# LukasHedegaard/continual-skeletons

Measured on AMD Instinct MI355X. Metric: clips/sec (ST-GCN clip forward, NTU-60 shape; CoST-GCN online step reported under costgcn_online), higher is better.
Workload: dtype f32

## Files before the change

### continual-skeletons_amd/csrc/gcn.hip

```cpp
#include <type_traits>

#include "mfma_core.h"
#include "gcn_params.h"


template <int MT, int NJ>
__global__ __launch_bounds__(NTHREADS, 2) void gcn_stage_kernel(const GcnParams p) {
    constexpr int NT = 16384 / MT;
    constexpr int WM = MT / 64;
    constexpr int TPC = NTHREADS / NT;
    constexpr int KPT = KC / TPC;
    extern __shared__ __attribute__((aligned(16))) float smem[];
    const int V = p.V, R = p.R, EW = p.ell_w;
    float *Wl = smem;
    float *Xa = Wl + R * KC * MT;
    float *Bx = Xa + R * KC * NT;
    float *Lv = Bx + KC * p.ldb;
    int *Ls = reinterpret_cast<int *>(Lv + 3 * V * EW * (p.adj_per_frame ? p.lds_frames : 1));

    const int tid = threadIdx.x, lane = tid & 63, wave = __builtin_amdgcn_readfirstlane(tid >> 6);
    const int wm = wave % WM, wn = wave / WM;
    const int l31 = lane & 31, kh = lane >> 5;
    const unsigned wid = xcd_contiguous_id(blockIdx.x, gridDim.x);
    const int m0 = (int)(wid % p.mtiles) * MT, q0 = (int)((wid / p.mtiles) % p.qtiles) * NT;
// ... 155 lines not shown
        for (int g = 0; g < 16; ++g) {
            const float v0 = relu_nan(acc[mi][0][g] + bb[mi][g] + rv[0][mi][g]);
            const float v1 = relu_nan(acc[mi][1][g] + bb[mi][g] + rv[1][mi][g]);
            const auto sw = __builtin_amdgcn_permlane32_swap(__float_as_uint(v0), __float_as_uint(v1), false, false);
            acc[mi][0][g] = __uint_as_float(sw[0]);
            acc[mi][1][g] = __uint_as_float(sw[1]);
        }
    const int qb = q0 + wn * 64 + lane;
    const bool qv = qb < Q;
    if (full) {
        if (qv) {
            const unsigned qo = 4u * (unsigned)qb;
#pragma unroll
            for (int mi = 0; mi < 2; ++mi)
#pragma unroll
                for (int g = 0; g < 16; ++g) {
                    float *orow = oseg + (int64_t)(rbase + mi * 32 + (g & 3) + 8 * (g >> 2)) * p.y_chan_stride;
                    st_lane(orow, qo, acc[mi][0][g]);
                    st_lane(orow + 4 * p.y_chan_stride, qo, acc[mi][1][g]);
                }
        }
    } else {
#pragma unroll
        for (int mi = 0; mi < 2; ++mi)
#pragma unroll
            for (int g = 0; g < 16; ++g) {
                const int row0 = rbase + mi * 32 + (g & 3) + 8 * (g >> 2);
                if (qv && row0 < p.Cout) oseg[(int64_t)row0 * p.y_chan_stride + qb] = acc[mi][0][g];
                if (qv && row0 + 4 < p.Cout) oseg[(int64_t)(row0 + 4) * p.y_chan_stride + qb] = acc[mi][1][g];
            }
    }
}

template <int MT, bool CONVRES, int KCG_, bool PLAIN = false, bool SPLIT = false>
__global__ __launch_bounds__(NTHREADS, 3) void gcn_stage_sparse2_kernel(const GcnParams p) {
    constexpr int NT = 16384 / MT;
    constexpr int WM = MT / 64;
    constexpr int R = PLAIN ? 1 : (CONVRES ? 4 : 3);
    constexpr int M4 = MT / 4;
    constexpr int WB = (R * KCG_ * M4 + NTHREADS - 1) / NTHREADS;
    constexpr int RPW = KCG_ / (NTHREADS / 64);
    constexpr int NJ = MT == 128 ? 3 : 5;
    constexpr int NS = KCG_ / 2;
    constexpr int NH = NS / 2;
    static_assert(KCG_ % 8 == 0, "a chunk is a whole number of rows per wave");
    extern __shared__ __attribute__((aligned(16))) float smem[];
    const int V = p.V;
    const int wsz = R * KCG_ * MT, bsz = KCG_ * p.ldb, bufsz = wsz + bsz;

    const int tid = threadIdx.x, lane = tid & 63, wave = __builtin_amdgcn_readfirstlane(tid >> 6);
    const int wm = wave % WM, wn = wave / WM;
    const int l31 = lane & 31, kh = lane >> 5;
    const unsigned wid = xcd_contiguous_id(blockIdx.x, gridDim.x);
    const int m0 = (int)(wid % p.mtiles) * MT, q0 = (int)((wid / p.mtiles) % p.qtiles) * NT;
    const int segks = (int)(wid / (p.mtiles * p.qtiles));
    const int seg = SPLIT ? segks / p.ksplit : segks, ks = SPLIT ? segks % p.ksplit : 0;
    const int cb = SPLIT ? ks * p.cper : 0;
    const int Q = p.frames * V;
    const int qend = min(q0 + NT, Q);
    const int ta = div_magic(q0, p.vmagic), tb = div_magic(qend - 1, p.vmagic);
    const int span = (tb - ta + 1) * V;
    int eoff[2][6];
    float eval[2][6];
    int ioff[2];
#pragma unroll
    for (int ni = 0; ni < 2; ++ni) {
        const int q = min(q0 + wn * 64 + ni * 32 + l31, Q - 1);
        const int t = div_magic(q, p.vmagic);
        const int w = q - t * V, fb = (t - ta) * V;
        ioff[ni] = fb + w;
#pragma unroll
        for (int e = 0; e < 6; ++e) {
            const int r = e < 2 ? e : 2, k = e < 2 ? 0 : e - 2;
            const bool have = !PLAIN && k < p.ell_cnt[r];
            const int idx = PLAIN ? 0 : (r * V + w) * p.ell_w + min(k, p.ell_w - 1);
            eoff[ni][e] = fb + (have ? p.ell_src[idx] : 0);
            eval[ni][e] = have ? p.ell_val[idx] : 0.f;
        }
    }

    f32x16 acc[2][2];
#pragma unroll
    for (int a = 0; a < 2; ++a)
#pragma unroll
        for (int b = 0; b < 2; ++b)
#pragma unroll
            for (int g = 0; g < 16; ++g) acc[a][b][g] = 0.f;

    const float *seg_base = p.x + (int64_t)seg * p.x_seg_stride;
    const float *wbase = p.w + m0 + (size_t)cb * p.Mpad;
    f32x4 wv[WB];
    unsigned wgo[WB], wlo[WB];
#pragma unroll
    for (int u = 0; u < WB; ++u) {
        const int e = min(u * NTHREADS + tid, R * KCG_ * M4 - 1);
        const int row = e / M4, m4 = e % M4;
        wgo[u] = (unsigned)(((row / KCG_) * p.CinPad + (row % KCG_)) * p.Mpad + m4 * 4);
        wlo[u] = (unsigned)(e * 4);
    }
    constexpr int NJ4 = (NJ + 3) / 4;
    float bv[RPW][NJ];
    f32x4 bv4[RPW][NJ4];
    unsigned bgo[NJ], blo[NJ];
#pragma unroll
    for (int u = 0; u < NJ; ++u) {
        const int j = min(u * 64 + lane, span - 1);
        bgo[u] = (unsigned)(ta * V + j);
        blo[u] = (unsigned)j;
    }
    const int nvec = (span + 3) / 4;
    const bool vec = ta * V + 4 * nvec <= Q && p.Cin >= KCG_;
    unsigned bgo4[NJ4], blo4[NJ4];
#pragma unroll
    for (int u = 0; u < NJ4; ++u) {
        const int i = min(u * 64 + lane, nvec - 1);
        bgo4[u] = (unsigned)(ta * V + 4 * i);
        blo4[u] = (unsigned)(4 * i);
    }
    auto issue_one = [&](auto vtag, int i, int c0) {
        constexpr bool VEC = decltype(vtag)::value;
        constexpr int NX = VEC ? NJ4 : NJ;
        if (i < WB) {
            wv[i] = *reinterpret_cast<const f32x4 *>(wbase + (size_t)c0 * p.Mpad + wgo[i]);
        } else {
            const int rr = (i - WB) / NX, u = (i - WB) % NX;
            const int c = min(cb + c0 + wave + rr * (NTHREADS / 64), p.Cin - 1);
            const float *row = seg_base + (int64_t)c * p.x_chan_stride;
            if (VEC) bv4[rr][u] = *reinterpret_cast<const f32x4u *>(row + bgo4[u]);
            else bv[rr][u] = row[bgo[u]];
        }
    };
    auto commit = [&](auto vtag, float *buf) {
        constexpr bool VEC = decltype(vtag)::value;
        float *Wl = buf, *Bx = buf + wsz;
#pragma unroll
        for (int u = 0; u < WB; ++u) *reinterpret_cast<f32x4 *>(Wl + wlo[u]) = wv[u];
#pragma unroll
        for (int rr = 0; rr < RPW; ++rr) {
            float *dst = Bx + (wave + rr * (NTHREADS / 64)) * p.ldb;
            if (VEC) {
#pragma unroll
                for (int u = 0; u < NJ4; ++u) *reinterpret_cast<f32x4 *>(dst + blo4[u]) = bv4[rr][u];
            } else {
#pragma unroll
                for (int u = 0; u < NJ; ++u) dst[blo[u]] = bv[rr][u];
            }
        }
    };
    const int offA = wm * 64 + l31;
    auto mfma_step = [&](const float *buf, int s) {
        const float *Wl = buf, *Bx = buf + wsz;
        const int kk = 2 * s + kh;
        const float *bx = Bx + kk * p.ldb;
        float b[R][2];
#pragma unroll
        for (int ni = 0; ni < 2; ++ni) {
            if constexpr (PLAIN) {
                b[0][ni] = bx[ioff[ni]];
            } else {
                const float x0 = bx[eoff[ni][0]];
// ... 5 lines not shown
                s2 = fmaf(eval[ni][5], bx[eoff[ni][5]], s2);
                b[2][ni] = s2;
                if (CONVRES) b[R - 1][ni] = bx[ioff[ni]];
            }
        }
#pragma unroll
        for (int r = 0; r < R; ++r) {
            const float *wr = Wl + (r * KCG_ + kk) * MT + offA;
            const float a0 = wr[0], a1 = wr[32];
            acc[0][0] = __builtin_amdgcn_mfma_f32_32x32x2f32(a0, b[r][0], acc[0][0], 0, 0, 0);
            acc[0][1] = __builtin_amdgcn_mfma_f32_32x32x2f32(a0, b[r][1], acc[0][1], 0, 0, 0);
            acc[1][0] = __builtin_amdgcn_mfma_f32_32x32x2f32(a1, b[r][0], acc[1][0], 0, 0, 0);
            acc[1][1] = __builtin_amdgcn_mfma_f32_32x32x2f32(a1, b[r][1], acc[1][1], 0, 0, 0);
        }
    };

    const int nchunks = (SPLIT ? min(p.CinPad - cb, p.cper) : p.CinPad) / KCG_;
    auto k_loop = [&](auto vtag) {
        constexpr int NLX = WB + RPW * (decltype(vtag)::value ? NJ4 : NJ);
#pragma unroll
        for (int i = 0; i < NLX; ++i) issue_one(vtag, i, 0);
        commit(vtag, smem);
        if (nchunks > 1) {
#pragma unroll
            for (int i = 0; i < NLX; ++i) issue_one(vtag, i, KCG_);
        }
        __syncthreads();
        for (int c = 0; c + 1 < nchunks; ++c) {
            float *cur = smem + (c & 1) * bufsz, *oth = smem + ((c & 1) ^ 1) * bufsz;
            commit(vtag, oth);
            const int cnext = min(c + 2, nchunks - 1) * KCG_;
            __builtin_amdgcn_s_setprio(1);
#pragma unroll
            for (int s = 0; s < NS; ++s) {
                if (s < NH) {
#pragma unroll
                    for (int i = s * NLX / NH; i < (s + 1) * NLX / NH; ++i) issue_one(vtag, i, cnext);
                    __builtin_amdgcn_sched_barrier(0);
                }
                mfma_step(cur, s);
            }
            __builtin_amdgcn_s_setprio(0);
            __syncthreads();
        }
    };
    if (vec) k_loop(std::true_type{});
    else k_loop(std::false_type{});
    const float *last = smem + ((nchunks - 1) & 1) * bufsz;
    const int rbase = m0 + wm * 64;
    const bool full = p.fast_epi && m0 + MT <= p.Cout;
    const unsigned kh4 = 4u * (unsigned)kh;
    float *oseg = SPLIT ? p.part + (int64_t)(seg * p.ksplit + ks) * p.Cout * p.y_chan_stride : p.y + (int64_t)seg * p.y_seg_stride;
    const int qb = q0 + wn * 64 + lane;
    const bool qv = qb < Q;
    float bb[2][16], rv[2][2][16];
    auto load_half = [&](int mi) {
        if (SPLIT) {
#pragma unroll
            for (int g = 0; g < 16; ++g) bb[mi][g] = rv[0][mi][g] = rv[1][mi][g] = 0.f;
        } else if (full) {
#pragma unroll
            for (int g = 0; g < 16; ++g) bb[mi][g] = ld_lane(p.bias + (rbase + mi * 32 + (g & 3) + 8 * (g >> 2)), kh4 * 4u);
#pragma unroll
            for (int ni = 0; ni < 2; ++ni) {
                const unsigned lo = 4u * (kh4 * (unsigned)p.x_chan_stride + (unsigned)min(q0 + wn * 64 + ni * 32 + l31, Q - 1));
#pragma unroll
                for (int g = 0; g < 16; ++g) {
                    const float *rrow = seg_base + (int64_t)(rbase + mi * 32 + (g & 3) + 8 * (g >> 2)) * p.x_chan_stride;
                    rv[ni][mi][g] = (CONVRES || PLAIN) ? 0.f : ld_lane(rrow, lo);
                }
            }
        } else {
#pragma unroll
            for (int g = 0; g < 16; ++g) bb[mi][g] = p.bias[rbase + mi * 32 + 4 * kh + (g & 3) + 8 * (g >> 2)];
#pragma unroll
            for (int ni = 0; ni < 2; ++ni) {
                const int qc = min(q0 + wn * 64 + ni * 32 + l31, Q - 1);
#pragma unroll
                for (int g = 0; g < 16; ++g) {
                    const int co = rbase + mi * 32 + 4 * kh + (g & 3) + 8 * (g >> 2);
                    rv[ni][mi][g] = (CONVRES || PLAIN) ? 0.f : seg_base[(int64_t)min(co, p.Cout - 1) * p.x_chan_stride + qc];
                }
            }
        }
    };
    auto finish_half = [&](int mi) {
#pragma unroll
        for (int g = 0; g < 16; ++g) {
            float v0 = acc[mi][0][g] + bb[mi][g] + rv[0][mi][g];
            float v1 = acc[mi][1][g] + bb[mi][g] + rv[1][mi][g];
            if (!PLAIN && !SPLIT) { v0 = relu_nan(v0); v1 = relu_nan(v1); }
            const auto sw = __builtin_amdgcn_permlane32_swap(__float_as_uint(v0), __float_as_uint(v1), false, false);
            acc[mi][0][g] = __uint_as_float(sw[0]);
            acc[mi][1][g] = __uint_as_float(sw[1]);
        }
        if (full) {
            if (qv) {
                const unsigned qo = 4u * (unsigned)qb;
#pragma unroll
                for (int g = 0; g < 16; ++g) {
                    float *orow = oseg + (int64_t)(rbase + mi * 32 + (g & 3) + 8 * (g >> 2)) * p.y_chan_stride;
                    st_lane(orow, qo, acc[mi][0][g]);
                    st_lane(orow + 4 * p.y_chan_stride, qo, acc[mi][1][g]);
                }
            }
        } else {
#pragma unroll
            for (int g = 0; g < 16; ++g) {
                const int row0 = rbase + mi * 32 + (g & 3) + 8 * (g >> 2);
                if (qv && row0 < p.Cout) oseg[(int64_t)row0 * p.y_chan_stride + qb] = acc[mi][0][g];
                if (qv && row0 + 4 < p.Cout) oseg[(int64_t)(row0 + 4) * p.y_chan_stride + qb] = acc[mi][1][g];
            }
        }
    };
#pragma unroll
    for (int s = 0; s < NS; ++s) mfma_step(last, s);
    load_half(0);
    finish_half(0);
    load_half(1);
    finish_half(1);
}

template <int MT, bool CONVRES, int KC2, int OCC>
__global__ __launch_bounds__(NTHREADS, OCC) void gcn_stage_dense_kernel(const GcnParams p) {
    constexpr int NT = 16384 / MT;
    constexpr int WM = MT / 64;
    constexpr int R = CONVRES ? 4 : 3;
    constexpr int M4 = MT / 4;
    constexpr int WB = R * KC2 * M4 / NTHREADS;
    constexpr int WBU = (R * KC2 * M4 + NTHREADS - 1) / NTHREADS;
    extern __shared__ __attribute__((aligned(16))) float smem[];
    const int V = p.V, FT = p.lds_frames, ldbx = p.ldb;
    float *Wl = smem;
    float *Xa = Wl + R * KC2 * MT;
    float *Bx = Xa + 3 * KC2 * NT;
    float *Ladj = Bx + KC2 * ldbx;

    const int tid = threadIdx.x, lane = tid & 63, wave = __builtin_amdgcn_readfirstlane(tid >> 6);
    const int wm = wave % WM, wn = wave / WM;
    const int l31 = lane & 31, kh = lane >> 5;
    const unsigned wid = xcd_contiguous_id(blockIdx.x, gridDim.x);
    const int m0 = (int)(wid % p.mtiles) * MT, qt = (int)((wid / p.mtiles) % p.qtiles);
    const int seg = (int)(wid / (p.mtiles * p.qtiles));
    const int Q = p.frames * V;
    const int ta = qt * FT, q0 = ta * V;
    const int fcnt = min(FT, p.frames - ta);
    const int ncol = fcnt * V;
    (void)WB;

    {
        const float *gv = p.ell_val + (int64_t)seg * p.adj_seg_stride;
        for (int e = tid; e < 3 * V * V; e += NTHREADS) Ladj[e] = gv[e];
    }
    f32x16 acc[2][2];
#pragma unroll
    for (int a = 0; a < 2; ++a)
#pragma unroll
        for (int b = 0; b < 2; ++b)
#pragma unroll
            for (int g = 0; g < 16; ++g) acc[a][b][g] = 0.f;

    const float *seg_base = p.x + (int64_t)seg * p.x_seg_stride;
    const float *wbase = p.w + m0;
    f32x4 wv[WBU];
// ... 153 lines not shown
                }
            }
        } else {
#pragma unroll
            for (int g = 0; g < 16; ++g) {
                const int row0 = rbase + mi * 32 + (g & 3) + 8 * (g >> 2);
                if (qv && row0 < p.Cout) oseg[(int64_t)row0 * p.y_chan_stride + qb] = acc[mi][0][g];
                if (qv && row0 + 4 < p.Cout) oseg[(int64_t)(row0 + 4) * p.y_chan_stride + qb] = acc[mi][1][g];
            }
        }
    }
}

__global__ __launch_bounds__(256) void gcn_reduce_kernel(const GcnParams p) {
    const int Q = p.frames * p.V;
    const int64_t i = (int64_t)blockIdx.x * 256 + threadIdx.x;
    if (i >= (int64_t)p.Cout * Q) return;
    const int co = (int)(i / Q), q = (int)(i - (int64_t)co * Q), seg = blockIdx.y;
    float s = 0.f;
    for (int ks = 0; ks < p.ksplit; ++ks) s += p.part[((int64_t)(seg * p.ksplit + ks) * p.Cout + co) * p.y_chan_stride + q];
    s += p.bias[co];
    if (p.res_mode == CSK_RES_IDENTITY) s += p.x[(int64_t)seg * p.x_seg_stride + (int64_t)co * p.x_chan_stride + q];
    p.y[(int64_t)seg * p.y_seg_stride + (int64_t)co * p.y_chan_stride + q] = relu_nan(s);
}

static int gcn_stage_setup(const float *x, float *y, const float *w, const float *bias, const int32_t *ell_src, const float *ell_val,
                           const int32_t *ell_cnt, int ell_w, int64_t adj_seg_stride, int adj_per_frame, int n_seg, int c_in, int c_out,
                           int frames, int V, int64_t x_seg_stride, int64_t x_chan_stride, int64_t y_seg_stride, int64_t y_chan_stride,
                           int res_mode, int ksplit, float *partial, GcnParams *out, size_t *lds_out, bool *sparse_out) {
    if (n_seg <= 0 || c_in <= 0 || c_out <= 0 || frames <= 0 || V < 2 || V > 64) CSK_FAIL("gcn_stage: bad dims");
    if (ell_w < 1 || ell_w > V) CSK_FAIL("gcn_stage: ell_w must be in [1, V]");
    if (res_mode != CSK_RES_IDENTITY && res_mode != CSK_RES_CONV) CSK_FAIL("gcn_stage: res_mode must be identity or conv");
    if (res_mode == CSK_RES_IDENTITY && c_in != c_out) CSK_FAIL("gcn_stage: identity residual needs c_in == c_out");
    for (int i = 0; i < 3; ++i)
        if (ell_cnt[i] < 0 || ell_cnt[i] > ell_w) CSK_FAIL("gcn_stage: ell_cnt[%d] out of range", i);
    GcnParams &p = *out;
    p = gcn_params(x, y, w, bias, ell_src, ell_val, ell_cnt, ell_w, adj_seg_stride, c_in, c_out, frames, V, x_seg_stride,
                   x_chan_stride, y_seg_stride, y_chan_stride, res_mode, partial);
    p.dense = adj_seg_stride != 0 && ell_w == V && ell_cnt[0] == V && ell_cnt[1] == V && ell_cnt[2] == V;
    p.adj_per_frame = adj_per_frame != 0;
    if (p.adj_per_frame && !p.dense) CSK_FAIL("gcn_stage: per-frame adjacency must be dense (ell_w == V, ell_cnt == V)");
    const bool big = (p.Mpad % 128) == 0;
    const int MT = big ? 128 : 64, NT = 16384 / MT;
    const int max_dt = (NT + V - 2) / V;
    p.ldb = round_up((max_dt + 1) * V, 4);
    p.lds_frames = max_dt + 1;
    const size_t lds = (size_t)(p.R * KC * MT + p.R * KC * NT + KC * p.ldb + 3 * V * ell_w * (1 + (p.adj_per_frame ? p.lds_frames : 1))) * sizeof(float);
    if (lds > 160 * 1024) CSK_FAIL("gcn_stage: LDS tile %zu B exceeds 160 KiB", lds);
    const int Q = frames * V;
    if ((int64_t)frames * V >= (1 << 26)) CSK_FAIL("gcn_stage: frames*V too large for 32-bit position arithmetic");
    p.qtiles = (Q + NT - 1) / NT; p.mtiles = p.Mpad / MT;
    if ((int64_t)p.qtiles * p.mtiles * n_seg >= (1ll << 31)) CSK_FAIL("gcn_stage: grid too large");
    const bool sparse = adj_seg_stride == 0 && ell_cnt[0] <= 1 && ell_cnt[1] <= 1 && ell_cnt[2] <= 4 && p.ldb <= (big ? 192 : 320) &&
                        !csk_diag_flag("CSK_GCN_GENERAL");
    if (ksplit > 1 && !sparse) CSK_FAIL("gcn_stage_splitk: split-K is built for the skeleton-sparse kernel (shared adjacency, <= 1/1/4 non-zeros per column)");
    p.ksplit = split_ranges(p.CinPad, c_in, ksplit, 8, &p.cper);
    *lds_out = lds; *sparse_out = sparse;
    return 0;
}

static bool gcn16_candidate(const GcnParams &p, bool sparse) { return sparse && p.ksplit == 1; }

enum { ROUTE_UNIT = 1000000, ROUTE_SPARSE2 = 1, ROUTE_TILE16 = 2, ROUTE_DENSE2 = 3, ROUTE_DENSE128 = 4, ROUTE_GENERAL = 5 };
enum { ROUTE_SPLIT = 1 << 30, ROUTE_SPLIT_MT128 = 1 << 29, ROUTE_SPLIT_CONVRES = 1 << 28, ROUTE_SPLIT_RANGES_SHIFT = 23, ROUTE_SPLIT_CPER_MASK = (1 << 23) - 1 };
static int gcn_stage_route(const GcnParams &p, bool sparse, int n_seg) {
    const bool big = (p.Mpad % 128) == 0;
    const int MT = big ? 128 : 64, NT = 16384 / MT, V = p.V;
    if (p.ksplit > 1) {
        if (p.cper / 8 > ROUTE_SPLIT_CPER_MASK) CSK_FAIL("gcn_stage_splitk: %d channels per range exceed the split launch", p.cper);
        return ROUTE_SPLIT | (big ? ROUTE_SPLIT_MT128 : 0) | (p.R == 4 ? ROUTE_SPLIT_CONVRES : 0) | ((p.ksplit - 1) << ROUTE_SPLIT_RANGES_SHIFT) |
               (p.cper / 8);
    }
    if (gcn16_candidate(p, sparse)) {
        if (const int tile = csk_gcn16_tile(p, n_seg)) return ROUTE_TILE16 * ROUTE_UNIT + tile;
    }
    if (sparse) return ROUTE_SPARSE2 * ROUTE_UNIT + MT * 10 + (p.R == 4 ? 1 : 0);
    if (p.dense) {
        if (const int d2 = csk_gcn_dense2_route(p, n_seg)) return ROUTE_DENSE2 * ROUTE_UNIT + d2;
    }
    if (big && p.dense && !p.adj_per_frame && V >= 4 && V <= 32 && NT / V >= 1 && p.frames * (int64_t)V >= 4) {
        const int ft = NT / V;
        if ((int64_t)((p.frames + ft - 1) / ft) * p.mtiles * n_seg >= (1ll << 31)) CSK_FAIL("gcn_stage: grid too large");
        return ROUTE_DENSE128 * ROUTE_UNIT + (p.R == 4 ? 1 : 0);
    }
    const int nj = (p.ldb + 63) / 64;
    if (nj > (big ? 4 : 6)) CSK_FAIL("gcn_stage: activation tile of %d positions per channel exceeds the staged maximum", p.ldb);
    return ROUTE_GENERAL * ROUTE_UNIT + MT * 10 + (big ? (nj <= 3 ? 3 : 4) : (nj <= 5 ? 5 : 6));
}

static int gcn_stage_impl(const float *x, float *y, const float *w, const float *bias, const int32_t *ell_src,
                          const float *ell_val, const int32_t *ell_cnt, int ell_w, int64_t adj_seg_stride,
                          int adj_per_frame,
                          int n_seg, int c_in, int c_out, int frames, int V, int64_t x_seg_stride,
                          int64_t x_chan_stride, int64_t y_seg_stride, int64_t y_chan_stride, int res_mode,
                          int ksplit, float *partial, void *stream) {
    if (!x || !y || !w || !bias || !ell_src || !ell_val || !ell_cnt) CSK_FAIL("gcn_stage: null pointer");
    GcnParams p;
    size_t lds;
    bool sparse;
    if (const int rc = gcn_stage_setup(x, y, w, bias, ell_src, ell_val, ell_cnt, ell_w, adj_seg_stride, adj_per_frame, n_seg, c_in, c_out, frames,
                                       V, x_seg_stride, x_chan_stride, y_seg_stride, y_chan_stride, res_mode, ksplit, partial, &p, &lds, &sparse))
        return rc;
    const bool big = (p.Mpad % 128) == 0;
    const int MT = big ? 128 : 64, NT = 16384 / MT;
    const int Q = frames * V;
    dim3 grid(p.qtiles * p.mtiles * n_seg);
    const int route = gcn_stage_route(p, sparse, n_seg);
    if (route < 0) return route;
    const bool split = (route & ROUTE_SPLIT) != 0;
    const int family = split ? ROUTE_SPARSE2 : route / ROUTE_UNIT;
    if (family == ROUTE_TILE16) return csk_launch_gcn16(p, n_seg, stream);
    if (family == ROUTE_SPARSE2) {
        const int R = p.R;
        size_t lds2;
        void (*k)(GcnParams);
        lds2 = 2 * (size_t)(R * 8 * MT + 8 * p.ldb) * sizeof(float);
        if (split) {
            const bool big2 = (route & ROUTE_SPLIT_MT128) != 0, convres = (route & ROUTE_SPLIT_CONVRES) != 0;
            const int ranges = ((route >> ROUTE_SPLIT_RANGES_SHIFT) & 31) + 1;
            if ((int64_t)p.qtiles * p.mtiles * n_seg * ranges >= (1ll << 31)) CSK_FAIL("gcn_stage: grid too large");
            grid = dim3(p.qtiles * p.mtiles * n_seg * ranges);
            k = big2 ? (convres ? gcn_stage_sparse2_kernel<128, true, 8, false, true> : gcn_stage_sparse2_kernel<128, false, 8, false, true>)
                     : (convres ? gcn_stage_sparse2_kernel<64, true, 8, false, true> : gcn_stage_sparse2_kernel<64, false, 8, false, true>);
        } else {
            k = big ? (R == 4 ? gcn_stage_sparse2_kernel<128, true, 8> : gcn_stage_sparse2_kernel<128, false, 8>)
                    : (R == 4 ? gcn_stage_sparse2_kernel<64, true, 8> : gcn_stage_sparse2_kernel<64, false, 8>);
        }
        const int e = csk_ensure_lds((const void *)k, lds2);
        if (e) return e;
        hipLaunchKernelGGL(k, grid, dim3(NTHREADS), lds2, (hipStream_t)stream, p);
        if (split) {
            if (const int e2 = (int)hipGetLastError()) return e2;
            const int64_t work = (int64_t)c_out * Q;
            hipLaunchKernelGGL(gcn_reduce_kernel, dim3((unsigned)((work + 255) / 256), n_seg), dim3(256), 0, (hipStream_t)stream, p);
        }
        return (int)hipGetLastError();
    }
    if (family == ROUTE_DENSE2) return csk_launch_gcn_dense2(p, n_seg, stream);
    if (family == ROUTE_DENSE128) {
        const int KC2 = 8;
        p.lds_frames = NT / V;
        int ldbx = round_up(p.lds_frames * V, 4);
        if ((ldbx / 4) % 2 == 0) ldbx += 4;
        p.ldb = ldbx;
        p.qtiles = (frames + p.lds_frames - 1) / p.lds_frames;
        const size_t ldsd = (size_t)(p.R * KC2 * MT + 3 * KC2 * NT + KC2 * ldbx + 3 * V * V) * sizeof(float);
        void (*kd)(GcnParams) = p.R == 4 ? gcn_stage_dense_kernel<128, true, 8, 3> : gcn_stage_dense_kernel<128, false, 8, 3>;
        if (const int e = csk_ensure_lds((const void *)kd, ldsd)) return e;
        hipLaunchKernelGGL(kd, dim3(p.qtiles * p.mtiles * n_seg), dim3(NTHREADS), ldsd, (hipStream_t)stream, p);
        return (int)hipGetLastError();
    }
    const int nj = route % 10;
    void (*kern)(GcnParams) = big ? (nj == 3 ? gcn_stage_kernel<128, 3> : gcn_stage_kernel<128, 4>)
                                  : (nj == 5 ? gcn_stage_kernel<64, 5> : gcn_stage_kernel<64, 6>);
    if (const int e = csk_ensure_lds((const void *)kern, lds)) return e;
    hipLaunchKernelGGL(kern, grid, dim3(NTHREADS), lds, (hipStream_t)stream, p);
    return (int)hipGetLastError();
}

extern "C" int csk_gcn_stage_f32(const float *x, float *y, const float *w, const float *bias, const int32_t *ell_src,
                                 const float *ell_val, const int32_t *ell_cnt, int ell_w, int64_t adj_seg_stride,
                                 int adj_per_frame,
                                 int n_seg, int c_in, int c_out, int frames, int V, int64_t x_seg_stride,
                                 int64_t x_chan_stride, int64_t y_seg_stride, int64_t y_chan_stride, int res_mode,
                                 void *stream) {
    return gcn_stage_impl(x, y, w, bias, ell_src, ell_val, ell_cnt, ell_w, adj_seg_stride, adj_per_frame, n_seg, c_in, c_out, frames,
                          V, x_seg_stride, x_chan_stride, y_seg_stride, y_chan_stride, res_mode, 1, nullptr, stream);
}

extern "C" int csk_gcn_stage_f32_tile(const float *x, const float *y, const int32_t *ell_cnt, int ell_w, int64_t adj_seg_stride,
                                      int adj_per_frame, int n_seg, int c_in, int c_out, int frames, int V, int64_t x_seg_stride,
                                      int64_t x_chan_stride, int64_t y_seg_stride, int64_t y_chan_stride, int res_mode) {
    if (!ell_cnt) CSK_FAIL("gcn_stage: null pointer");
    GcnParams p;
    size_t lds;
    bool sparse;
    if (const int rc = gcn_stage_setup(x, const_cast<float *>(y), nullptr, nullptr, nullptr, nullptr, ell_cnt, ell_w, adj_seg_stride, adj_per_frame,
                                       n_seg, c_in, c_out, frames, V, x_seg_stride, x_chan_stride, y_seg_stride, y_chan_stride, res_mode, 1,
                                       nullptr, &p, &lds, &sparse))
        return rc;
    return gcn16_candidate(p, sparse) ? csk_gcn16_tile(p, n_seg) : 0;
}

extern "C" int csk_gcn_stage_f32_route(const float *x, const float *y, const float *ell_val, const int32_t *ell_cnt, int ell_w,
                                       int64_t adj_seg_stride, int adj_per_frame, int n_seg, int c_in, int c_out, int frames, int V,
                                       int64_t x_seg_stride, int64_t x_chan_stride, int64_t y_seg_stride, int64_t y_chan_stride,
                                       int res_mode) {
    if (!ell_cnt) CSK_FAIL("gcn_stage: null pointer");
    GcnParams p;
    size_t lds;
    bool sparse;
    if (const int rc = gcn_stage_setup(x, const_cast<float *>(y), nullptr, nullptr, nullptr, ell_val, ell_cnt, ell_w, adj_seg_stride, adj_per_frame,
                                       n_seg, c_in, c_out, frames, V, x_seg_stride, x_chan_stride, y_seg_stride, y_chan_stride, res_mode, 1,
                                       nullptr, &p, &lds, &sparse))
        return rc;
    return gcn_stage_route(p, sparse, n_seg);
}

static int gcn_splitk_args(int ksplit, const float *partial) {
    if (ksplit < 1 || ksplit > 32 || (ksplit > 1 && !partial)) CSK_FAIL("gcn_stage_splitk: ksplit must be in [1, 32] and needs a partial-sum buffer");
    return 0;
}

extern "C" int csk_gcn_stage_splitk_f32_route(const float *x, const float *y, const float *ell_val, const int32_t *ell_cnt, int ell_w, int n_seg,
                                              int c_in, int c_out, int frames, int V, int64_t x_seg_stride, int64_t x_chan_stride,
                                              int64_t y_seg_stride, int64_t y_chan_stride, int res_mode, int ksplit, const float *partial) {
    if (const int rc = gcn_splitk_args(ksplit, partial)) return rc;
    if (!ell_cnt) CSK_FAIL("gcn_stage: null pointer");
    GcnParams p;
    size_t lds;
    bool sparse;
    if (const int rc = gcn_stage_setup(x, const_cast<float *>(y), nullptr, nullptr, nullptr, ell_val, ell_cnt, ell_w, 0, 0, n_seg, c_in, c_out, frames,
                                       V, x_seg_stride, x_chan_stride, y_seg_stride, y_chan_stride, res_mode, ksplit, const_cast<float *>(partial),
                                       &p, &lds, &sparse))
        return rc;
    return gcn_stage_route(p, sparse, n_seg);
}

extern "C" int csk_gcn_stage_splitk_f32(const float *x, float *y, const float *w, const float *bias, const int32_t *ell_src,
                                        const float *ell_val, const int32_t *ell_cnt, int ell_w, int n_seg, int c_in, int c_out,
                                        int frames, int V, int64_t x_seg_stride, int64_t x_chan_stride, int64_t y_seg_stride,
                                        int64_t y_chan_stride, int res_mode, int ksplit, float *partial, void *stream) {
    if (const int rc = gcn_splitk_args(ksplit, partial)) return rc;
    return gcn_stage_impl(x, y, w, bias, ell_src, ell_val, ell_cnt, ell_w, 0, 0, n_seg, c_in, c_out, frames, V, x_seg_stride,
                          x_chan_stride, y_seg_stride, y_chan_stride, res_mode, ksplit, partial, stream);
}


extern "C" int csk_conv1x1_f32(const float *x, float *y, const float *w, const float *bias, int n_seg, int c_in, int c_out,
                               int frames, int V, int64_t x_seg_stride, int64_t x_chan_stride, int64_t y_seg_stride,
                               int64_t y_chan_stride, void *stream) {
    if (!x || !y || !w || !bias) CSK_FAIL("conv1x1: null pointer");
    if (n_seg <= 0 || c_in <= 0 || c_out <= 0 || frames <= 0 || V < 2 || V > 64) CSK_FAIL("conv1x1: bad dims");
    if ((int64_t)frames * V >= (1 << 26)) CSK_FAIL("conv1x1: frames*V too large for 32-bit position arithmetic");
    const int32_t no_adjacency[3] = {0, 0, 0};
    GcnParams p = gcn_params(x, y, w, bias, nullptr, nullptr, no_adjacency, 1, 0, c_in, c_out, frames, V, x_seg_stride, x_chan_stride,
                             y_seg_stride, y_chan_stride, CSK_RES_NONE, nullptr);
    p.R = 1;
    const bool big = (p.Mpad % 128) == 0;
    const int MT = big ? 128 : 64, NT = 16384 / MT;
    const int max_dt = (NT + V - 2) / V;
    p.ldb = round_up((max_dt + 1) * V, 4);
    if (p.ldb > (big ? 192 : 320)) CSK_FAIL("conv1x1: activation tile of %d positions exceeds the staged maximum", p.ldb);
    const int Q = frames * V;
    p.qtiles = (Q + NT - 1) / NT; p.mtiles = p.Mpad / MT;
    if ((int64_t)p.qtiles * p.mtiles * n_seg >= (1ll << 31)) CSK_FAIL("conv1x1: grid too large");
    constexpr int KCP = 16;
    const size_t lds = 2 * (size_t)(KCP * MT + KCP * p.ldb) * sizeof(float);
    void (*k)(GcnParams) = big ? gcn_stage_sparse2_kernel<128, false, KCP, true> : gcn_stage_sparse2_kernel<64, false, KCP, true>;
    if (const int e = csk_ensure_lds((const void *)k, lds)) return e;
    hipLaunchKernelGGL(k, dim3(p.qtiles * p.mtiles * n_seg), dim3(NTHREADS), lds, (hipStream_t)stream, p);
    return (int)hipGetLastError();
}
```

### continual-skeletons_amd/csrc/gcn_params.h

```cpp
#pragma once
#include <stdint.h>

#include "mfma_core.h"

struct GcnParams {
    const float *x, *w, *bias;
    float *y;
    const int32_t *ell_src;
    const float *ell_val;
    int ell_cnt[3];
    int ell_w;
    int64_t adj_seg_stride, x_seg_stride, x_chan_stride, y_seg_stride, y_chan_stride;
    int Cin, CinPad, Cout, Mpad, frames, V, R, res_mode, ldb;
    unsigned vmagic, mtiles, qtiles;
    int dense;
    int adj_per_frame;
    int lds_frames;
    int fast_epi;
    int ksplit, cper;
    float *part;
    int x_ring_slots, x_ring_slot0, y_ring_slots, y_ring_slot0;
};

inline GcnParams gcn_params(const float *x, float *y, const float *w, const float *bias, const int32_t *ell_src, const float *ell_val,
                            const int32_t *ell_cnt, int ell_w, int64_t adj_seg_stride, int c_in, int c_out, int frames, int V, int64_t x_seg_stride,
                            int64_t x_chan_stride, int64_t y_seg_stride, int64_t y_chan_stride, int res_mode, float *part) {
    GcnParams p = {};
    p.x = x; p.w = w; p.bias = bias; p.y = y; p.ell_src = ell_src; p.ell_val = ell_val;
    for (int i = 0; i < 3; ++i) p.ell_cnt[i] = ell_cnt[i];
    p.ell_w = ell_w; p.adj_seg_stride = adj_seg_stride;
    p.x_seg_stride = x_seg_stride; p.x_chan_stride = x_chan_stride; p.y_seg_stride = y_seg_stride; p.y_chan_stride = y_chan_stride;
    p.Cin = c_in; p.CinPad = round_up(c_in, CSK_CPAD); p.Cout = c_out; p.Mpad = round_up(c_out, CSK_MT);
    p.frames = frames; p.V = V; p.R = res_mode == CSK_RES_CONV ? 4 : 3; p.res_mode = res_mode;
    p.vmagic = vmagic_of(V);
    p.fast_epi = x_chan_stride < (1ll << 27) && y_chan_stride < (1ll << 27);
    p.x_ring_slots = p.y_ring_slots = 1 << 30; p.x_ring_slot0 = p.y_ring_slot0 = 0;
    p.ksplit = 1; p.cper = p.CinPad; p.part = part;
    return p;
}

int csk_launch_gcn_dense2(GcnParams p, int n_seg, void *stream);
int csk_gcn_dense2_route(const GcnParams &p, int n_seg);

int csk_launch_gcn16(GcnParams p, int n_seg, void *stream);
int csk_gcn16_tile(const GcnParams &p, int n_seg);
```

### continual-skeletons_amd/native.py

```python
import ctypes as C
import os

import torch

_HERE = os.path.dirname(os.path.abspath(__file__))
LIB_PATH = os.path.join(_HERE, "libcskel_hip.so")
ABI_VERSION = 16

_p, _i, _l = C.c_void_p, C.c_int, C.c_int64
SIGNATURES = {
    "csk_abi_version": [],
    "csk_stream_overlap_probe": [C.c_void_p, C.c_void_p, C.c_int, C.POINTER(C.c_float)],
    "csk_gcn_stage_f32": [_p, _p, _p, _p, _p, _p, _p, _i, _l, _i, _i, _i, _i, _i, _i, _l, _l, _l, _l, _i, _p],
    "csk_gcn_stage_f32_tile": [_p, _p, _p, _i, _l, _i, _i, _i, _i, _i, _i, _l, _l, _l, _l, _i],
    "csk_gcn_stage_f32_route": [_p, _p, _p, _p, _i, _l, _i, _i, _i, _i, _i, _i, _l, _l, _l, _l, _i],
    "csk_gcn_stage_splitk_f32": [_p, _p, _p, _p, _p, _p, _p, _i, _i, _i, _i, _i, _i, _l, _l, _l, _l, _i, _i, _p, _p],
    "csk_gcn_stage_splitk_f32_route": [_p, _p, _p, _p, _i, _i, _i, _i, _i, _i, _l, _l, _l, _l, _i, _i, _p],
    "csk_tcn_stage_f32": [_p, _p, _p, _p, _p, _p, _i, _i, _i, _i, _i, _i, _i, _i, _i, _i, _i, _i, _i, _p],
    "csk_tcn_stage_wino_f32": [_p, _p, _p, _p, _p, _p, _i, _i, _i, _i, _i, _i, _i, _i, _i, _i, _i, _i, _i, _p, _p],
    "csk_tcn_stage_wino_ext_f32": [_p, _p, _p, _p, _p, _p, _i, _i, _i, _i, _i, _i, _i, _i, _i, _i, _i, _i, _i, _p, _p],
    "csk_tcn_stage_wino_valid_f32": [_p, _p, _p, _p, _p, _p, _i, _i, _i, _i, _i, _i, _i, _i, _i, _i, _i, _i, _i, _p, _p],
    "csk_tcn_stage_wino_valid_res_f32": [_p, _p, _p, _p, _p, _i, _i, _i, _i, _i, _i, _i, _i, _i, _i, _i, _i, _i, _p, _p],
    "csk_block_few_channels_f32": [_p, _p, _p, _p, _p, _p, _i, _p, _p, _p, _i, _i, _i, _i, _i, _i, _i, _p],
    "csk_tcn_stage_splitk_f32": [_p, _p, _p, _p, _p, _p, _i, _i, _i, _i, _i, _i, _i, _i, _i, _i, _i, _i, _i, _i, _p, _p],
    "csk_conv1x1_f32": [_p, _p, _p, _p, _i, _i, _i, _i, _i, _l, _l, _l, _l, _p],
    "csk_tcn_stage_bf16x3": [_p, _p, _p, _p, _p, _p, _i, _i, _i, _i, _i, _i, _i, _i, _i, _i, _i, _i, _i, _p],
    "csk_gcn_stage_bf16x3": [_p, _p, _p, _p, _p, _p, _p, _p, _i, _i, _i, _i, _i, _i, _i, _p],
    "csk_input_norm_f32": [_p, _p, _p, _p, _i, _i, _i, _i, _i, _l, _l, _p],
    "csk_pool_fc_f32": [_p, _p, _p, _p, _p, _i, _i, _i, _i, _i, _p],
    "csk_fc_f32": [_p, _p, _p, _p, _i, _i, _i, _p],
    "csk_pool_scaled_f32": [_p, _p, _i, _i, _i, _i, C.c_float, _p],
    "csk_agcn_attention_f32": [_p, _p, _p, _p, _i, _i, _i, _i, _l, _l, _i, _l, _p],
    "csk_agcn_embed_attention_f32": [_p, _p, _p, _p, _p, _p, _i, _i, _i, _i, _i, _i, _l, _l, _p],
    "csk_agcn_stage_framewise_f32": [_p, _p, _p, _p, _p, _p, _p, _i, _i, _i, _i, _i, _i, _l, _l, _l, _l, _i, _p],
    "csk_agcn_stage_framewise_f32_route": [_p, _i, _i, _i, _i, _i, _i, _l, _l, _i],
    "csk_tcn_step_f32": [_p, _i, _i, _i, _i, _p, _p, _i, _i, _i, _p, _p, _p, _i, _i, _i, _i, _l, _i, _i, _i, _i, _i, _p, _p],
    "csk_tcn_step_f32_tile": [_i, _i, _i, _i, _i, _i, _i, _l, _i, _i, _i, _i],
    "csk_tcn_step_bf16x3": [_p, _i, _i, _i, _i, _p, _p, _i, _i, _i, _p, _p, _p, _i, _i, _i, _i, _l, _i, _i, _i, _i, _p],
    "csk_tcn_step_bf16x3_tile": [_i, _i, _l],
    "csk_co_stack_step_f32": [_i, _p, _i, _i, _l, _p],
    "csk_co_block_step_f32": [_p, _i, _i, _i, _p, _p, _p, _p, _p, _i, _i, _p, _i, _i, _p, _p, _i, _i, _p, _i, _i, _i, _i, _i, _l, _p],
    "csk_co_spatial_pool_f32": [_p, _p, _i, _i, _i, _l, _p],
    "csk_co_window_mean_f32": [_p, _p, _l, _i, _i, _i, _p],
    "csk_co_head_step_f32": [_p, _p, _p, _p, _p, _p, _i, _i, _i, _l, _i, _i, _i, _i, _i, _p],
    "csk_co_head_clip_f32": [_p, _i, _i, _p, _i, _i, _i, _p, _p, _p, _p, _i, _i, _i, _i, _i, _p],
    "csk_input_norm_frames_f32": [_p, _p, _i, _p, _p, _i, _i, _i, _i, _l, _p],
    "csk_derive_modality_f32": [_p, _p, _i, _p, _i, _i, _i, _i, _i, _p],
    "csk_derive_modality_frames_f32": [_p, _p, _i, _i, _p, _p, _p, _i, _i, _i, _i, _i, _p],
    "csk_prenorm_f32": [_p, _p, _i, _i, _i, _i, _i, _i, _i, _i, _p],
    "csk_prenorm_frames_f32": [_p, _p, _i, _p, _p, _i, _i, _i, _i, _i, _i, _i, _i, _p],
    "csk_select_people_f32": [_p, _p, _i, _i, _i, _i, _i, _p],
    "csk_select_people_frames_f32": [_p, _p, _i, _i, _i, _i, _i, _p],
    "csk_ntu_intake_f32": [_p, _p, _i, _i, _i, _i, _i, _i, _p],

    "csk_fuse_rank_f32": [_p, _i, _i, _i, _i, _l, _l, _p, _p, _p, _p],
    "csk_co_plan_create": [_i, _p, _p, _i, _i, _i, _i, _i, _l, _p, _p, _i, _p, _p, _i, _i, _p, _p],
    "csk_co_plan_destroy": [_p],
    "csk_co_plan_update_weights": [_p, _i, _p, _p, _p, _p, _p],
    "csk_co_plan_set_fusion": [_p, _i],
    "csk_co_plan_set_delays": [_p, _i, _p],
    "csk_co_plan_cycle": [_p, C.POINTER(C.c_int64), _i, _p, _i, _p, _p, _p, _p, _p],
    "csk_co_scrub_streams_f32": [_p, _i, _p, _i, _i, _p],
    "csk_co_move_streams_f32": [_p, _i, _p, _l, _p, _i, _i, _i, _p],
    "csk_co_prime_pack_f32": [_p, _i, _p, _l, _i, _i, _i, _p],
    "csk_str_unit_f32": [_p, _p, _p, _l, _p, _p, _p, _p, _p, _p, _p, _i, _i, _i, _i, _i, _l, _l, _l, _l, _p],
}
RESTYPES = {"csk_co_plan_create": C.c_void_p, "csk_co_plan_destroy": None}

# ... 87 lines not shown
```

### include/cskel.h

```cpp
#ifndef CSKEL_H
#define CSKEL_H

#include <stdint.h>

#ifdef __cplusplus
extern "C" {
#endif

#define CSK_ABI_VERSION 16
#define CSK_KC 8
#define CSK_CPAD 16
#define CSK_MT 64

#define CSK_RES_NONE 0
#define CSK_RES_IDENTITY 1
#define CSK_RES_CONV 2

int csk_abi_version(void);
const char *csk_last_error(void);

int csk_stream_overlap_probe(void *stream_a, void *stream_b, int spin_us, float *ratio);

int csk_gcn_stage_f32(const float *x, float *y, const float *w, const float *bias,
                      const int32_t *ell_src, const float *ell_val, const int32_t *ell_cnt,
                      int ell_w, int64_t adj_seg_stride, int adj_per_frame,
                      int n_seg, int c_in, int c_out, int frames, int V,
                      int64_t x_seg_stride, int64_t x_chan_stride,
                      int64_t y_seg_stride, int64_t y_chan_stride,
                      int res_mode, void *stream);

int csk_gcn_stage_f32_tile(const float *x, const float *y, const int32_t *ell_cnt, int ell_w, int64_t adj_seg_stride,
                           int adj_per_frame, int n_seg, int c_in, int c_out, int frames, int V,
                           int64_t x_seg_stride, int64_t x_chan_stride, int64_t y_seg_stride, int64_t y_chan_stride,
                           int res_mode);

int csk_gcn_stage_f32_route(const float *x, const float *y, const float *ell_val, const int32_t *ell_cnt, int ell_w,
                            int64_t adj_seg_stride, int adj_per_frame, int n_seg, int c_in, int c_out, int frames, int V,
                            int64_t x_seg_stride, int64_t x_chan_stride, int64_t y_seg_stride, int64_t y_chan_stride,
                            int res_mode);

int csk_gcn_stage_splitk_f32(const float *x, float *y, const float *w, const float *bias, const int32_t *ell_src,
                             const float *ell_val, const int32_t *ell_cnt, int ell_w, int n_seg, int c_in, int c_out,
                             int frames, int V, int64_t x_seg_stride, int64_t x_chan_stride, int64_t y_seg_stride,
                             int64_t y_chan_stride, int res_mode, int ksplit, float *partial, void *stream);

int csk_gcn_stage_splitk_f32_route(const float *x, const float *y, const float *ell_val, const int32_t *ell_cnt, int ell_w, int n_seg,
                                   int c_in, int c_out, int frames, int V, int64_t x_seg_stride, int64_t x_chan_stride,
                                   int64_t y_seg_stride, int64_t y_chan_stride, int res_mode, int ksplit, const float *partial);

int csk_tcn_stage_f32(const float *y, const float *w, const float *x_res, const float *w_res,
                      const float *bias, float *out,
                      int n_seg, int c, int c_out, int t_in, int V, int k, int stride, int pad,
                      int res_mode, int c_res, int t_res, int res_off, int relu, void *stream);

int csk_tcn_stage_wino_f32(const float *y, const float *w, const float *x_res, const float *w_res,
                           const float *bias, float *out,
                           int n_seg, int c, int c_out, int t_in, int V, int k, int stride, int pad,
                           int res_mode, int c_res, int t_res, int res_off, int relu, const float *w_wino, void *stream);

int csk_tcn_stage_wino_ext_f32(const float *y, const float *w, const float *x_res, const float *w_res,
                               const float *bias, float *out,
                               int n_seg, int c, int c_out, int t_in, int V, int k, int stride, int pad,
                               int res_mode, int c_res, int t_res, int res_off, int relu, const float *w_wino_ext, void *stream);

int csk_tcn_stage_wino_valid_f32(const float *y, const float *w, const float *x_res, const float *w_res,
                                 const float *bias, float *out,
                                 int n_seg, int c, int c_out, int t_in, int V, int k, int stride, int pad,
                                 int res_mode, int c_res, int t_res, int res_off, int relu, const float *w_wino, void *stream);

int csk_tcn_stage_wino_valid_res_f32(const float *y, const float *x_res, const float *w_res, const float *bias, float *out,
                                     int n_seg, int c, int c_out, int t_in, int V, int k, int stride, int pad,
                                     int res_mode, int c_res, int t_res, int res_off, int relu, const float *w_wino, void *stream);

int csk_block_few_channels_f32(const float *x, const float *gcn_w, const float *gcn_bias, const int32_t *ell_src,
                               const float *ell_val, const int32_t *ell_cnt, int ell_w, const float *tcn_w,
                               const float *tcn_bias, float *out, int n_seg, int c_in, int c_mid, int c_out, int t_in,
                               int V, int pad, void *stream);

int csk_tcn_stage_splitk_f32(const float *y, const float *w, const float *x_res, const float *w_res,
                             const float *bias, float *out,
                             int n_seg, int c, int c_out, int t_in, int V, int k, int stride, int pad,
                             int res_mode, int c_res, int t_res, int res_off, int relu, int ksplit, float *partial,
                             void *stream);

int csk_conv1x1_f32(const float *x, float *y, const float *w, const float *bias, int n_seg, int c_in, int c_out,
                    int frames, int V, int64_t x_seg_stride, int64_t x_chan_stride, int64_t y_seg_stride,
                    int64_t y_chan_stride, void *stream);

int csk_tcn_stage_bf16x3(const float *y, const void *w_split, const float *x_res, const void *w_res_split,
// ... 197 lines not shown
```

Before: 4344.

## Tile GCN columns across segment boundaries to remove per-segment tail tiles

The sparse GCN kernel can now tile the column dimension over all segments laid end to end. Tiles that straddle a segment boundary jump addresses by the segment stride, so each segment no longer ends in a partly filled column tile. This cuts the grid size and wasted MFMA work when frames*V is not a multiple of the tile width. The cost is extra index arithmetic and conditional offsets in loads and stores, plus overflow guards that fall back to per-segment tiling. A tile-count query entry point and a diagnostic flag to turn it off are also added.

```diff
diff --git a/continual-skeletons_amd/csrc/gcn.hip b/continual-skeletons_amd/csrc/gcn.hip
--- a/continual-skeletons_amd/csrc/gcn.hip
+++ b/continual-skeletons_amd/csrc/gcn.hip
@@ -231,12 +231,19 @@
     const int wm = wave % WM, wn = wave / WM;
     const int l31 = lane & 31, kh = lane >> 5;
     const unsigned wid = xcd_contiguous_id(blockIdx.x, gridDim.x);
-    const int m0 = (int)(wid % p.mtiles) * MT, q0 = (int)((wid / p.mtiles) % p.qtiles) * NT;
+    const int m0 = (int)(wid % p.mtiles) * MT, qflat = (int)((wid / p.mtiles) % p.qtiles) * NT;
     const int segks = (int)(wid / (p.mtiles * p.qtiles));
-    const int seg = SPLIT ? segks / p.ksplit : segks, ks = SPLIT ? segks % p.ksplit : 0;
+    const int ks = SPLIT ? segks % p.ksplit : 0;
     const int cb = SPLIT ? ks * p.cper : 0;
     const int Q = p.frames * V;
-    const int qend = min(q0 + NT, Q);
+    const bool flat = !SPLIT && p.flat_nseg > 0;
+    const int fseg = flat ? (int)((unsigned)qflat / (unsigned)Q) : 0;
+    const int seg = SPLIT ? segks / p.ksplit : (flat ? fseg : segks);
+    const int q0 = qflat - fseg * Q;
+    const int Qe = flat ? (p.flat_nseg - fseg) * Q : Q;
+    const int qend = min(q0 + NT, Qe);
+    const bool cross = !SPLIT && qend > Q;
+    const int64_t xjump = cross ? p.x_seg_stride - Q : 0, yjump = cross ? p.y_seg_stride - Q : 0;
     const int ta = div_magic(q0, p.vmagic), tb = div_magic(qend - 1, p.vmagic);
     const int span = (tb - ta + 1) * V;
     int eoff[2][6];
@@ -244,7 +251,7 @@
     int ioff[2];
 #pragma unroll
     for (int ni = 0; ni < 2; ++ni) {
-        const int q = min(q0 + wn * 64 + ni * 32 + l31, Q - 1);
+        const int q = min(q0 + wn * 64 + ni * 32 + l31, Qe - 1);
         const int t = div_magic(q, p.vmagic);
         const int w = q - t * V, fb = (t - ta) * V;
         ioff[ni] = fb + w;
@@ -284,7 +291,8 @@
 #pragma unroll
     for (int u = 0; u < NJ; ++u) {
         const int j = min(u * 64 + lane, span - 1);
-        bgo[u] = (unsigned)(ta * V + j);
+        const int pos = ta * V + j;
+        bgo[u] = (unsigned)pos + (pos >= Q ? (unsigned)xjump : 0u);
         blo[u] = (unsigned)j;
     }
     const int nvec = (span + 3) / 4;
@@ -396,7 +404,8 @@
     const unsigned kh4 = 4u * (unsigned)kh;
     float *oseg = SPLIT ? p.part + (int64_t)(seg * p.ksplit + ks) * p.Cout * p.y_chan_stride : p.y + (int64_t)seg * p.y_seg_stride;
     const int qb = q0 + wn * 64 + lane;
-    const bool qv = qb < Q;
+    const bool qv = qb < Qe;
+    const int64_t qbj = qb >= Q ? yjump : 0;
     float bb[2][16], rv[2][2][16];
     auto load_half = [&](int mi) {
         if (SPLIT) {
@@ -407,7 +416,8 @@
             for (int g = 0; g < 16; ++g) bb[mi][g] = ld_lane(p.bias + (rbase + mi * 32 + (g & 3) + 8 * (g >> 2)), kh4 * 4u);
 #pragma unroll
             for (int ni = 0; ni < 2; ++ni) {
-                const unsigned lo = 4u * (kh4 * (unsigned)p.x_chan_stride + (unsigned)min(q0 + wn * 64 + ni * 32 + l31, Q - 1));
+                const int qc = min(q0 + wn * 64 + ni * 32 + l31, Qe - 1);
+                const unsigned lo = 4u * (kh4 * (unsigned)p.x_chan_stride + (unsigned)qc + (qc >= Q ? (unsigned)xjump : 0u));
 #pragma unroll
                 for (int g = 0; g < 16; ++g) {
                     const float *rrow = seg_base + (int64_t)(rbase + mi * 32 + (g & 3) + 8 * (g >> 2)) * p.x_chan_stride;
@@ -419,11 +429,12 @@
             for (int g = 0; g < 16; ++g) bb[mi][g] = p.bias[rbase + mi * 32 + 4 * kh + (g & 3) + 8 * (g >> 2)];
 #pragma unroll
             for (int ni = 0; ni < 2; ++ni) {
-                const int qc = min(q0 + wn * 64 + ni * 32 + l31, Q - 1);
+                const int qc = min(q0 + wn * 64 + ni * 32 + l31, Qe - 1);
+                const int64_t qcj = qc + (qc >= Q ? xjump : 0);
 #pragma unroll
                 for (int g = 0; g < 16; ++g) {
                     const int co = rbase + mi * 32 + 4 * kh + (g & 3) + 8 * (g >> 2);
-                    rv[ni][mi][g] = (CONVRES || PLAIN) ? 0.f : seg_base[(int64_t)min(co, p.Cout - 1) * p.x_chan_stride + qc];
+                    rv[ni][mi][g] = (CONVRES || PLAIN) ? 0.f : seg_base[(int64_t)min(co, p.Cout - 1) * p.x_chan_stride + qcj];
                 }
             }
         }
@@ -440,7 +451,7 @@
         }
         if (full) {
             if (qv) {
-                const unsigned qo = 4u * (unsigned)qb;
+                const unsigned qo = 4u * ((unsigned)qb + (unsigned)qbj);
 #pragma unroll
                 for (int g = 0; g < 16; ++g) {
                     float *orow = oseg + (int64_t)(rbase + mi * 32 + (g & 3) + 8 * (g >> 2)) * p.y_chan_stride;
@@ -452,8 +463,8 @@
 #pragma unroll
             for (int g = 0; g < 16; ++g) {
                 const int row0 = rbase + mi * 32 + (g & 3) + 8 * (g >> 2);
-                if (qv && row0 < p.Cout) oseg[(int64_t)row0 * p.y_chan_stride + qb] = acc[mi][0][g];
-                if (qv && row0 + 4 < p.Cout) oseg[(int64_t)(row0 + 4) * p.y_chan_stride + qb] = acc[mi][1][g];
+                if (qv && row0 < p.Cout) oseg[(int64_t)row0 * p.y_chan_stride + qb + qbj] = acc[mi][0][g];
+                if (qv && row0 + 4 < p.Cout) oseg[(int64_t)(row0 + 4) * p.y_chan_stride + qb + qbj] = acc[mi][1][g];
             }
         }
     };
@@ -713,11 +724,22 @@
     p.qtiles = (Q + NT - 1) / NT; p.mtiles = p.Mpad / MT;
     if ((int64_t)p.qtiles * p.mtiles * n_seg >= (1ll << 31)) CSK_FAIL("gcn_stage: grid too large");
     const bool sparse = adj_seg_stride == 0 && ell_cnt[0] <= 1 && ell_cnt[1] <= 1 && ell_cnt[2] <= 4 && p.ldb <= (big ? 192 : 320) &&
-                        !csk_diag_flag("CSK_GCN_GENERAL");
+                        (!csk_diag_flag("CSK_GCN_GENERAL") || csk_diag_int("CSK_GCN_GENERAL") == 2);
     if (ksplit > 1 && !sparse) CSK_FAIL("gcn_stage_splitk: split-K is built for the skeleton-sparse kernel (shared adjacency, <= 1/1/4 non-zeros per column)");
     p.ksplit = split_ranges(p.CinPad, c_in, ksplit, 8, &p.cper);
     *lds_out = lds; *sparse_out = sparse;
     return 0;
+}
+
+static int64_t gcn_flat_tiling(GcnParams &p, int n_seg, int NT) {
+    const int64_t Q = (int64_t)p.frames * p.V, lim = 1ll << 30;
+    const bool fits = p.x_seg_stride >= Q && p.y_seg_stride >= Q && n_seg * Q < lim &&
+                      4 * p.x_chan_stride + p.x_seg_stride + Q + NT < lim && 4 * p.y_chan_stride + p.y_seg_stride + Q + NT < lim &&
+                      p.x_chan_stride >= 0 && p.y_chan_stride >= 0;
+    const bool flat = n_seg > 1 && Q >= NT && fits && csk_diag_int("CSK_GCN_GENERAL") != 2;
+    p.flat_nseg = flat ? n_seg : 0;
+    p.qtiles = (unsigned)(((flat ? n_seg * Q : Q) + NT - 1) / NT);
+    return flat ? (int64_t)p.qtiles : (int64_t)p.qtiles * n_seg;
 }
 
 static bool gcn16_candidate(const GcnParams &p, bool sparse) { return sparse && p.ksplit == 1; }
@@ -784,6 +806,7 @@
             k = big2 ? (convres ? gcn_stage_sparse2_kernel<128, true, 8, false, true> : gcn_stage_sparse2_kernel<128, false, 8, false, true>)
                      : (convres ? gcn_stage_sparse2_kernel<64, true, 8, false, true> : gcn_stage_sparse2_kernel<64, false, 8, false, true>);
         } else {
+            grid = dim3((unsigned)(gcn_flat_tiling(p, n_seg, NT) * p.mtiles));
             k = big ? (R == 4 ? gcn_stage_sparse2_kernel<128, true, 8> : gcn_stage_sparse2_kernel<128, false, 8>)
                     : (R == 4 ? gcn_stage_sparse2_kernel<64, true, 8> : gcn_stage_sparse2_kernel<64, false, 8>);
         }
@@ -856,6 +879,25 @@
                                        nullptr, &p, &lds, &sparse))
         return rc;
     return gcn_stage_route(p, sparse, n_seg);
+}
+
+extern "C" int csk_gcn_stage_f32_tiles(const float *x, const float *y, const float *ell_val, const int32_t *ell_cnt, int ell_w,
+                                       int64_t adj_seg_stride, int adj_per_frame, int n_seg, int c_in, int c_out, int frames, int V,
+                                       int64_t x_seg_stride, int64_t x_chan_stride, int64_t y_seg_stride, int64_t y_chan_stride,
+                                       int res_mode) {
+    if (!ell_cnt) CSK_FAIL("gcn_stage: null pointer");
+    GcnParams p;
+    size_t lds;
+    bool sparse;
+    if (const int rc = gcn_stage_setup(x, const_cast<float *>(y), nullptr, nullptr, nullptr, ell_val, ell_cnt, ell_w, adj_seg_stride, adj_per_frame,
+                                       n_seg, c_in, c_out, frames, V, x_seg_stride, x_chan_stride, y_seg_stride, y_chan_stride, res_mode, 1,
+                                       nullptr, &p, &lds, &sparse))
+        return rc;
+    const int route = gcn_stage_route(p, sparse, n_seg);
+    if (route < 0) return route;
+    if (route / ROUTE_UNIT != ROUTE_SPARSE2) return 0;
+    const int64_t tiles = gcn_flat_tiling(p, n_seg, 16384 / (route % ROUTE_UNIT / 10));
+    return (int)tiles | (p.flat_nseg ? 1 << 30 : 0);
 }
 
 static int gcn_splitk_args(int ksplit, const float *partial) {
@@ -906,10 +948,11 @@
     const int Q = frames * V;
     p.qtiles = (Q + NT - 1) / NT; p.mtiles = p.Mpad / MT;
     if ((int64_t)p.qtiles * p.mtiles * n_seg >= (1ll << 31)) CSK_FAIL("conv1x1: grid too large");
+    const int64_t tiles = gcn_flat_tiling(p, n_seg, NT);
     constexpr int KCP = 16;
     const size_t lds = 2 * (size_t)(KCP * MT + KCP * p.ldb) * sizeof(float);
     void (*k)(GcnParams) = big ? gcn_stage_sparse2_kernel<128, false, KCP, true> : gcn_stage_sparse2_kernel<64, false, KCP, true>;
     if (const int e = csk_ensure_lds((const void *)k, lds)) return e;
-    hipLaunchKernelGGL(k, dim3(p.qtiles * p.mtiles * n_seg), dim3(NTHREADS), lds, (hipStream_t)stream, p);
+    hipLaunchKernelGGL(k, dim3((unsigned)(tiles * p.mtiles)), dim3(NTHREADS), lds, (hipStream_t)stream, p);
     return (int)hipGetLastError();
 }
diff --git a/continual-skeletons_amd/csrc/gcn_params.h b/continual-skeletons_amd/csrc/gcn_params.h
--- a/continual-skeletons_amd/csrc/gcn_params.h
+++ b/continual-skeletons_amd/csrc/gcn_params.h
@@ -19,6 +19,7 @@
     int fast_epi;
     int ksplit, cper;
     float *part;
+    int flat_nseg;
     int x_ring_slots, x_ring_slot0, y_ring_slots, y_ring_slot0;
 };
 
diff --git a/continual-skeletons_amd/native.py b/continual-skeletons_amd/native.py
--- a/continual-skeletons_amd/native.py
+++ b/continual-skeletons_amd/native.py
@@ -14,6 +14,7 @@
     "csk_gcn_stage_f32": [_p, _p, _p, _p, _p, _p, _p, _i, _l, _i, _i, _i, _i, _i, _i, _l, _l, _l, _l, _i, _p],
     "csk_gcn_stage_f32_tile": [_p, _p, _p, _i, _l, _i, _i, _i, _i, _i, _i, _l, _l, _l, _l, _i],
     "csk_gcn_stage_f32_route": [_p, _p, _p, _p, _i, _l, _i, _i, _i, _i, _i, _i, _l, _l, _l, _l, _i],
+    "csk_gcn_stage_f32_tiles": [_p, _p, _p, _p, _i, _l, _i, _i, _i, _i, _i, _i, _l, _l, _l, _l, _i],
     "csk_gcn_stage_splitk_f32": [_p, _p, _p, _p, _p, _p, _p, _i, _i, _i, _i, _i, _i, _l, _l, _l, _l, _i, _i, _p, _p],
     "csk_gcn_stage_splitk_f32_route": [_p, _p, _p, _p, _i, _i, _i, _i, _i, _i, _l, _l, _l, _l, _i, _i, _p],
     "csk_tcn_stage_f32": [_p, _p, _p, _p, _p, _p, _i, _i, _i, _i, _i, _i, _i, _i, _i, _i, _i, _i, _i, _p],
diff --git a/include/cskel.h b/include/cskel.h
--- a/include/cskel.h
+++ b/include/cskel.h
@@ -35,6 +35,11 @@
                            int res_mode);
 
 int csk_gcn_stage_f32_route(const float *x, const float *y, const float *ell_val, const int32_t *ell_cnt, int ell_w,
+                            int64_t adj_seg_stride, int adj_per_frame, int n_seg, int c_in, int c_out, int frames, int V,
+                            int64_t x_seg_stride, int64_t x_chan_stride, int64_t y_seg_stride, int64_t y_chan_stride,
+                            int res_mode);
+
+int csk_gcn_stage_f32_tiles(const float *x, const float *y, const float *ell_val, const int32_t *ell_cnt, int ell_w,
                             int64_t adj_seg_stride, int adj_per_frame, int n_seg, int c_in, int c_out, int frames, int V,
                             int64_t x_seg_stride, int64_t x_chan_stride, int64_t y_seg_stride, int64_t y_chan_stride,
                             int res_mode);
```

New measurement: 4361, median of 6. About the same (+0.4%).
